# andi611/ZeroSpeech-TTS-without-T

Measured on AMD Instinct MI355X. Metric: mel-frames/sec (train_ae, seg_len=128, enc_size=1024), higher is better.
Workload: dtype bf16

## Files before the change

### include/zs_amd.h

```cpp
#ifndef ZS_AMD_H
#define ZS_AMD_H
#include <stddef.h>
#include <stdint.h>

#ifdef __cplusplus
extern "C" {
#endif

#define ZS_ABI_VERSION 1

enum { ZS_F32 = 0, ZS_BF16 = 1 };
enum { ZS_OK = 0, ZS_EINVAL = -1, ZS_ELAUNCH = -2, ZS_EWORKSPACE = -3 };
enum { ZS_PAD_ZERO = 0, ZS_PAD_REFLECT = 1 };
enum { ZS_ACT_NONE = 0, ZS_ACT_LRELU = 1, ZS_ACT_SIGMOID = 2, ZS_ACT_TANH = 3 };
enum { ZS_STORE_ROWS = 0, ZS_STORE_SPLIT2 = 1 };
enum { ZS_RES_NONE = 0, ZS_RES_IDENTITY = 1, ZS_RES_AVGPOOL2 = 2, ZS_RES_UPSAMPLE2 = 3 };

int zs_abi_version(void);
const char* zs_last_error(void);
int zs_set_option(const char* key, int value);

typedef struct {
  int32_t dtype;
  const void* A; int64_t lda; int64_t a_batch_stride;
  int32_t B, T_in, T_out;
  int32_t taps, stride, pad_left, pad_mode, gather;
  int32_t cin_pad;
  const void* W; int64_t ldw;
  int32_t N, n_pad;
  const float* bias;
  const float* pre_vec; int64_t pre_vec_ld; const int64_t* vec_idx;
  int32_t act; float slope;
  const void* dact_src; int64_t dact_ld;
  const void* add_src; int64_t add_ld; int32_t add_f32;
  void* out; int64_t ldc; int32_t out_f32; int32_t out_cols; int32_t store_mode;
  void* out2; int64_t ldc2; int32_t out2_cols; int32_t store_mode2;
  const float* vec2; int64_t vec2_ld;
  int32_t groups; int64_t a_gstride, w_gstride, out_gstride, bias_gstride;
  float* colsum; int64_t colsum_ld; int32_t colsum_col0;
  int32_t colsum_post;
  const int32_t* lengths; int32_t pad_right;
  int32_t w_in, w_out, taps_h;
} ZsGemmConv;
int zs_gemm_conv(const ZsGemmConv* p, void* stream);

typedef struct {
  int32_t dtype;
  const void* dY; int64_t ldy; int32_t y_cols;
  const void* X; int64_t ldx; int64_t x_batch_stride; int32_t x_cols;
  int32_t B, T_in, T_out;
  int32_t taps, stride, pad_left, pad_mode;
  int32_t Cout, Cin;
  float* dW; int64_t so, si, sj;
  float* db;
  int32_t co_split2; int32_t accumulate;
  int32_t splits;
  void* workspace; size_t workspace_bytes;
  int32_t w_in, w_out, taps_h;
} ZsGemmWgrad;
size_t zs_gemm_wgrad_workspace_bytes(const ZsGemmWgrad* p);
int zs_gemm_wgrad(const ZsGemmWgrad* p, void* stream);

typedef struct {
  int32_t dtype;
  const float* W; int64_t so, si, sj;
  int32_t Cout, Cin, taps;
  int32_t transpose, co_split2;
  int32_t inner_pad;
  void* dst; int64_t ldw;
  int32_t n_rows, n_cols, row_offset, col_offset;
  const int32_t* row_perm;
} ZsPackWeight;
int zs_pack_weight(const ZsPackWeight* p, void* stream);
int zs_pack_weight_batch(const ZsPackWeight* jobs, int32_t n, int32_t max_blocks, void* stream);

typedef struct {
  const float* src; float* dst;
  int32_t len, src_stride, dst_stride;
} ZsVecCopy;
int zs_copy_vec_batch(const ZsVecCopy* jobs, int32_t n, void* stream);

// ... 320 lines not shown
```

### zerospeech-tts-without-t_amd/csrc/zs_gemm.hip

```cpp
#include <stdlib.h>

#include <atomic>
#include <mutex>

#include "zs_common.h"

namespace {

constexpr int BM = 128, BN = 128, NT = 256;
constexpr int ROWB = 128;
constexpr int PITCH = 144;
constexpr int TILE_BYTES = BM * PITCH;

__device__ const uint4 zs_zero_line[8] = {};

__device__ __forceinline__ int xcd_remap(int bid, int nwg) {
  const int q = nwg >> 3, r = nwg & 7, xcd = bid & 7;
  return (xcd < r ? xcd * (q + 1) : r * (q + 1) + (xcd - r) * q) + (bid >> 3);
}

__device__ __forceinline__ int conv_src_row(int gather, int pad_mode, int stride, int pad_left, int T_in, int t,
                                            int j, bool& ok) {
  if (gather == 0) {
    int s = t * stride + j - pad_left;
// ... 513 lines not shown
  gemm_epilogue<T, NT, MI>(p, acc, reinterpret_cast<float*>(smem), M, m0, n0, wm, wn, tid, g);
}

constexpr int RBM = 256, RNT = 512;
constexpr int RSTAGE = (RBM + BN) * 128;
constexpr int RING_LDS = 3 * RSTAGE;
typedef __attribute__((ext_vector_type(4))) unsigned u32x4_t;

template <typename T, int PP>
__global__ __launch_bounds__(RNT, 2) void gemm_conv_ring_kernel(const ZsGemmConv p) {
  const Geom2 g2 = make_geom2(p.w_in, p.w_out, p.taps_h, p.T_in);
  constexpr int EPS = 16 / (int)sizeof(T);
  constexpr int KC = ROWB / (int)sizeof(T);
  extern __shared__ __attribute__((aligned(16))) unsigned char smem[];
  const int tid = threadIdx.x, lane = tid & 63, wave = __builtin_amdgcn_readfirstlane(tid >> 6);
  const int wm = wave >> 1, wn = wave & 1;
  const int g = blockIdx.z;
  const T* __restrict__ A = (const T*)p.A + (int64_t)g * p.a_gstride;
  const T* __restrict__ W = (const T*)p.W + (int64_t)g * p.w_gstride;
  const int M = p.B * p.T_out;
  const int ntn = (p.N + BN - 1) / BN;
  const int ntm = (M + RBM - 1) / RBM;
  const int wg = xcd_remap(blockIdx.x, ntm * ntn);
  constexpr int GM = 4;
  const int per_group = GM * ntn;
  const int grp = wg / per_group;
  const int gm = min(GM, ntm - grp * GM);
  const int in_g = wg - grp * per_group;
  const int m0 = (grp * GM + in_g % gm) * RBM, n0 = (in_g / gm) * BN;

  const int lrow = lane >> 3, slot = lane & 7;
  int rb[4], rt[4], lseg[4];
#pragma unroll
  for (int i = 0; i < 4; ++i) {
    const int r = wave * 32 + i * 8 + lrow;
    lseg[i] = slot ^ ((r >> 1) & 7);
    const int m = m0 + r;
    conv_row_setup(p, m, M, rb[i], rt[i]);
  }
  const int chunks_per_tap = p.cin_pad / KC;
  const T* zline = reinterpret_cast<const T*>(zs_zero_line);
  const T *pa0, *pa1, *pa2, *pa3;
  int inc0, inc1, inc2, inc3;
#define ZS_SET_TAP(i, ptr, inc)                                                                         \
  {                                                                                                     \
    bool ok = false; int srow = 0;                                                                      \
    if (rb[i] >= 0) srow = conv_src_row_g(p.gather, p.pad_mode, p.stride, p.pad_left, conv_row_tin(p, rb[i]), rt[i], tap, ok, g2); \
    ptr = ok ? (A + (int64_t)conv_row_b(p, rb[i]) * p.a_batch_stride + (int64_t)srow * p.lda + lseg[i] * EPS) : (zline + lseg[i] * EPS); \
    inc = ok ? KC : 0;                                                                                  \
  }
  const int wr0 = wave * 16 + lrow, wr1 = wave * 16 + 8 + lrow;
  const T* pw0 = W + (int64_t)(n0 + wr0) * p.ldw + (slot ^ ((wr0 >> 1) & 7)) * EPS;
  const T* pw1 = W + (int64_t)(n0 + wr1) * p.ldw + (slot ^ ((wr1 >> 1) & 7)) * EPS;
  const int nk = p.taps * chunks_per_tap;
  int tap = 0, cit = 0;
  { ZS_SET_TAP(0, pa0, inc0) ZS_SET_TAP(1, pa1, inc1) ZS_SET_TAP(2, pa2, inc2) ZS_SET_TAP(3, pa3, inc3) }
  typedef __attribute__((address_space(1))) const void* gptr_t;
  typedef __attribute__((address_space(3))) void* lptr_t;
  auto dma_piece = [&](int stage, int i) {
    unsigned char* da = smem + stage * RSTAGE + wave * 4096;
    unsigned char* db = smem + stage * RSTAGE + RBM * 128 + wave * 2048;
    if (i == 0) __builtin_amdgcn_global_load_lds((gptr_t)pa0, (lptr_t)(da), 16, 0, 0);
    else if (i == 1) __builtin_amdgcn_global_load_lds((gptr_t)pa1, (lptr_t)(da + 1024), 16, 0, 0);
    else if (i == 2) __builtin_amdgcn_global_load_lds((gptr_t)pa2, (lptr_t)(da + 2048), 16, 0, 0);
    else if (i == 3) __builtin_amdgcn_global_load_lds((gptr_t)pa3, (lptr_t)(da + 3072), 16, 0, 0);
    else if (i == 4) __builtin_amdgcn_global_load_lds((gptr_t)pw0, (lptr_t)(db), 16, 0, 0);
    else __builtin_amdgcn_global_load_lds((gptr_t)pw1, (lptr_t)(db + 1024), 16, 0, 0);
  };
  auto dma_advance = [&]() {
    pw0 += KC; pw1 += KC;
    if (++cit == chunks_per_tap) {
      cit = 0; ++tap;
      if (tap < p.taps) { ZS_SET_TAP(0, pa0, inc0) ZS_SET_TAP(1, pa1, inc1) ZS_SET_TAP(2, pa2, inc2) ZS_SET_TAP(3, pa3, inc3) }
    } else {
      pa0 += inc0; pa1 += inc1; pa2 += inc2; pa3 += inc3;
    }
  };
  auto dma = [&](int stage) {
#pragma unroll
    for (int i = 0; i < 6; ++i) dma_piece(stage, i);
    dma_advance();
  };
#undef ZS_SET_TAP

  f32x16 acc[2][2];
#pragma unroll
  for (int i = 0; i < 2; ++i)
#pragma unroll
    for (int j = 0; j < 2; ++j)
#pragma unroll
      for (int r = 0; r < 16; ++r) acc[i][j][r] = 0.f;

  const int frow = lane & 31, fh = lane >> 5, fx = (frow >> 1) & 7;
  const unsigned lds0 = (unsigned)(uintptr_t)(__attribute__((address_space(3))) unsigned char*)smem;
  const unsigned a_lane = lds0 + (unsigned)((wm * 64 + frow) * 128);
  const unsigned b_lane = lds0 + (unsigned)(RBM * 128 + (wn * 64 + frow) * 128);
// ... 592 lines not shown
          asm volatile("ds_read_b64_tr_b16 %0, %1" : "=v"(rb[st][t][hb]) : "v"(xa + off));
        }
    asm volatile("s_waitcnt lgkmcnt(0)" ::: "memory");
    __builtin_amdgcn_sched_barrier(0);
#pragma unroll
    for (int st = 0; st < 2; ++st) {
      uint4 fa[2], fb[2];
#pragma unroll
      for (int t = 0; t < 2; ++t) {
        fa[t] = make_uint4(ra[st][t][0].x, ra[st][t][0].y, ra[st][t][1].x, ra[st][t][1].y);
        fb[t] = make_uint4(rb[st][t][0].x, rb[st][t][0].y, rb[st][t][1].x, rb[st][t][1].y);
      }
#pragma unroll
      for (int mi = 0; mi < 2; ++mi)
#pragma unroll
        for (int ni = 0; ni < 2; ++ni)
          acc[mi][ni] = __builtin_amdgcn_mfma_f32_32x32x16_bf16(__builtin_bit_cast(bf16x8, fa[mi]), __builtin_bit_cast(bf16x8, fb[ni]),
                                                                acc[mi][ni], 0, 0, 0);
    }
  }
};

template <typename T>
__global__ __launch_bounds__(NT, 2) void gemm_wgrad_kernel(const ZsGemmWgrad p, int ci_tiles, int rows_per_split,
                                                          int cout_r, int cin_r) {
  const Geom2 g2 = make_geom2(p.w_in, p.w_out, p.taps_h, p.T_in);
  constexpr int EPS = 16 / (int)sizeof(T);
  constexpr int SPR = 128 / EPS;
  constexpr int LPT = (WK * SPR) / NT;
  constexpr int PITCHW = WFrag<T>::PITCHW;
  constexpr int TILEW = WK * PITCHW;
  extern __shared__ __attribute__((aligned(16))) unsigned char smem[];
  unsigned char* sY = smem;
  unsigned char* sX = smem + 2 * TILEW;

  const int tid = threadIdx.x, lane = tid & 63, wave = tid >> 6;
  const int wm = wave >> 1, wn = wave & 1;
  const int per_co = p.taps * ci_tiles;
  const int tiles = ((cout_r / 128) * per_co);
  const int vid = xcd_remap(blockIdx.x, gridDim.x);
  const int split = vid / tiles, tile = vid - split * tiles;
  const int cot = tile / per_co;
  const int rem = tile - cot * per_co;
  const int tap = rem / ci_tiles, cit = rem - tap * ci_tiles;
  const int co0 = cot * 128, ci0 = cit * 128;
  const int M = p.B * p.T_out;
  const int nsplit = gridDim.x / tiles;
  const int mbeg = split * rows_per_split;
  const int mend = min(M, mbeg + rows_per_split);
  const T* __restrict__ dY = (const T*)p.dY;
  const T* __restrict__ X = (const T*)p.X;

  int lrow[LPT], lseg[LPT], lb[LPT], lt[LPT];
#pragma unroll
  for (int i = 0; i < LPT; ++i) {
    const int idx = tid + NT * i;
    lrow[i] = idx / SPR; lseg[i] = idx - lrow[i] * SPR;
    const int m = mbeg + lrow[i];
    lb[i] = m / p.T_out; lt[i] = m - lb[i] * p.T_out;
  }
  uint4 vy[LPT], vx[LPT];
  const bool do_bias = (p.db != nullptr) && tap == 0 && cit == 0;
  float bsum[LPT][EPS];
#pragma unroll
  for (int i = 0; i < LPT; ++i)
#pragma unroll
    for (int e = 0; e < EPS; ++e) bsum[i][e] = 0.f;
  auto gload = [&](int mb) {
#pragma unroll
    for (int i = 0; i < LPT; ++i) {
// ... 72 lines not shown
  float* sC = reinterpret_cast<float*>(smem);
  __syncthreads();
#pragma unroll
  for (int mi = 0; mi < 2; ++mi)
#pragma unroll
    for (int ni = 0; ni < 2; ++ni)
#pragma unroll
      for (int r = 0; r < 16; ++r) {
        const int row = wm * 64 + mi * 32 + (r & 3) + 8 * (r >> 2) + 4 * (lane >> 5);
        const int col = wn * 64 + ni * 32 + (lane & 31);
        sC[row * CPITCH + col] = acc[mi][ni][r];
      }
  __syncthreads();
  const int cg = tid & 15, rr0 = tid >> 4;
#pragma unroll 1
  for (int it = 0; it < 8; ++it) {
    const int row = rr0 + 16 * it;
    const float4 x0 = *reinterpret_cast<const float4*>(sC + row * CPITCH + cg * 8);
    const float4 x1 = *reinterpret_cast<const float4*>(sC + row * CPITCH + cg * 8 + 4);
    float* d = slab + ((int64_t)(co0 + row) * p.taps + tap) * cin_r + ci0 + cg * 8;
    *reinterpret_cast<float4*>(d) = x0;
    *reinterpret_cast<float4*>(d + 4) = x1;
  }
}

#define ZS_DSRT(dst, addr, off) asm volatile("ds_read_b64_tr_b16 %0, %1 offset:" #off : "=v"(dst) : "v"(addr))
#define ZS_WP_READ_A(base)                                                                        \
  ZS_DSRT(ya00, sa0, base + 0);    ZS_DSRT(yb00, sa0, base + 512);  ZS_DSRT(ya01, sa1, base + 0);    ZS_DSRT(yb01, sa1, base + 512);  \
  ZS_DSRT(ya10, sa0, base + 2048); ZS_DSRT(yb10, sa0, base + 2560); ZS_DSRT(ya11, sa1, base + 2048); ZS_DSRT(yb11, sa1, base + 2560); \
  ZS_DSRT(ya20, sa0, base + 4096); ZS_DSRT(yb20, sa0, base + 4608); ZS_DSRT(ya21, sa1, base + 4096); ZS_DSRT(yb21, sa1, base + 4608); \
  ZS_DSRT(ya30, sa0, base + 6144); ZS_DSRT(yb30, sa0, base + 6656); ZS_DSRT(ya31, sa1, base + 6144); ZS_DSRT(yb31, sa1, base + 6656);
#define ZS_WP_READ_B(x, sbx)                                                                      \
  ZS_DSRT(x##a0, sbx, 0);    ZS_DSRT(x##b0, sbx, 512);  ZS_DSRT(x##a1, sbx, 2048); ZS_DSRT(x##b1, sbx, 2560); \
  ZS_DSRT(x##a2, sbx, 4096); ZS_DSRT(x##b2, sbx, 4608); ZS_DSRT(x##a3, sbx, 6144); ZS_DSRT(x##b3, sbx, 6656);
#define ZS_WP_MMA(alo, ahi, blo, bhi, c)                                                          \
  c = __builtin_amdgcn_mfma_f32_32x32x16_bf16(__builtin_bit_cast(bf16x8, make_uint4(alo.x, alo.y, ahi.x, ahi.y)), \
                                               __builtin_bit_cast(bf16x8, make_uint4(blo.x, blo.y, bhi.x, bhi.y)), c, 0, 0, 0)
#define ZS_WP_DMA(cond, src, dst)                                                                 \
  __builtin_amdgcn_sched_barrier(0);                                                              \
  if (cond) __builtin_amdgcn_global_load_lds((gptr_t)(src), (lptr_t)(dst), 16, 0, 0);             \
  __builtin_amdgcn_sched_barrier(0);
#define ZS_WP_QUAD(c0, c1, x, cond, src0, dst0, src1, dst1)                                        \
  __builtin_amdgcn_s_setprio(1);                                                                  \
  ZS_WP_MMA(ya00, yb00, x##a0, x##b0, c0); ZS_WP_MMA(ya01, yb01, x##a0, x##b0, c1);               \
  ZS_WP_DMA(cond, src0, dst0)                                                                     \
  ZS_WP_MMA(ya10, yb10, x##a1, x##b1, c0); ZS_WP_MMA(ya11, yb11, x##a1, x##b1, c1); ZS_WP_MMA(ya20, yb20, x##a2, x##b2, c0); \
// ... 192 lines not shown
      for (int r = 0; r < 16; ++r) {
        const int ro = (r & 3) + 8 * (r >> 2);
        sC[(rbase + ro) * CPITCH + cb] = c000[r];            sC[(rbase + 32 + ro) * CPITCH + cb] = c001[r];
        sC[(rbase + ro) * CPITCH + cb + 32] = c010[r];       sC[(rbase + 32 + ro) * CPITCH + cb + 32] = c011[r];
        sC[(rbase + 64 + ro) * CPITCH + cb] = c100[r];       sC[(rbase + 96 + ro) * CPITCH + cb] = c101[r];
        sC[(rbase + 64 + ro) * CPITCH + cb + 32] = c110[r];  sC[(rbase + 96 + ro) * CPITCH + cb + 32] = c111[r];
      }
    }
    __syncthreads();
    const int cg = tid & 15, rr0 = tid >> 4;
#pragma unroll 1
    for (int it = 0; it < 8; ++it) {
      const int row = rr0 + 32 * it;
      const float4 x0 = *reinterpret_cast<const float4*>(sC + row * CPITCH + cg * 8);
      const float4 x1 = *reinterpret_cast<const float4*>(sC + row * CPITCH + cg * 8 + 4);
      float* d = slab + ((int64_t)(co0 + row) * p.taps + tap) * cin_r + ci0 + h * 128 + cg * 8;
      *reinterpret_cast<float4*>(d) = x0;
      *reinterpret_cast<float4*>(d + 4) = x1;
    }
    __syncthreads();
  }
}

__global__ __launch_bounds__(256) void wgrad_reduce_kernel(const ZsGemmWgrad p, int splits, int cout_r, int cin_r) {
  const int cin4 = (p.Cin + 3) >> 2;
  const int64_t total = (int64_t)p.Cout * p.taps * cin4;
  const int64_t idx = (int64_t)blockIdx.x * blockDim.x + threadIdx.x;
  if (idx >= total) return;
  const int c4 = (int)(idx % cin4);
  const int64_t rowi = idx / cin4;
  const int j = (int)(rowi % p.taps);
  const int co = (int)(rowi / p.taps);
  const int half = p.Cout >> 1;
  const int cop = p.co_split2 ? ((co & 1) * half + (co >> 1)) : co;
  const int64_t sstride = (int64_t)cout_r * p.taps * cin_r;
  const float* ws = (const float*)p.workspace + ((int64_t)cop * p.taps + j) * cin_r + c4 * 4;
  float4 acc = make_float4(0.f, 0.f, 0.f, 0.f);
  int k = 0;
  for (; k + 8 <= splits; k += 8) {
    float4 v[8];
#pragma unroll
    for (int u = 0; u < 8; ++u) v[u] = *reinterpret_cast<const float4*>(ws + (int64_t)(k + u) * sstride);
#pragma unroll
    for (int u = 0; u < 8; ++u) { acc.x += v[u].x; acc.y += v[u].y; acc.z += v[u].z; acc.w += v[u].w; }
  }
  for (; k < splits; ++k) {
    const float4 v = *reinterpret_cast<const float4*>(ws + (int64_t)k * sstride);
    acc.x += v.x; acc.y += v.y; acc.z += v.z; acc.w += v.w;
  }
  const float r[4] = {acc.x, acc.y, acc.z, acc.w};
  float* d = p.dW + (int64_t)co * p.so + (int64_t)j * p.sj;
#pragma unroll
  for (int e = 0; e < 4; ++e) {
    const int ci = c4 * 4 + e;
    if (ci < p.Cin) {
      float* q = d + (int64_t)ci * p.si;
      *q = p.accumulate ? (*q + r[e]) : r[e];
    }
  }
  if (p.db != nullptr && c4 == 0 && j == 0) {
    const float* bs = (const float*)p.workspace + (int64_t)splits * sstride + cop;
    float t = 0.f;
    for (int q2 = 0; q2 < splits; ++q2) t += bs[(int64_t)q2 * cout_r];
    p.db[co] = p.accumulate ? (p.db[co] + t) : t;
  }
}

int env_int(const char* name, int dflt) { const char* e = getenv(name); return e ? atoi(e) : dflt; }
struct Knob {
  std::atomic<int> v{-1};
  const char* env; int dflt;
  Knob(const char* e, int d) : env(e), dflt(d) {}
  int get() {
    int x = v.load(std::memory_order_relaxed);
    if (x < 0) { x = env_int(env, dflt); if (x < 0) x = 0; v.store(x, std::memory_order_relaxed); }
    return x;
  }
  int set(int nv) { const int old = get(); v.store(nv < 0 ? 0 : nv, std::memory_order_relaxed); return old; }
};
Knob g_dma64("ZS_GEMM_DMA64", 1);
Knob g_dma64_max_tiles("ZS_GEMM_DMA64_MAX_TILES", 256);
Knob g_wgrad_p8("ZS_WGRAD_P8", 1);
Knob g_wgrad_wgs("ZS_WGRAD_WGS", 256);
Knob g_wgrad_wgs128("ZS_WGRAD_WGS128", 448);
Knob g_wgrad_slab_cost("ZS_WGRAD_SLAB_COST", 13);
Knob g_wgrad_waste("ZS_WGRAD_P8_WASTE", 135);

struct WgradPlan { int p8, splits, tile, co_tiles, ci_tiles, cout_r, cin_r, rows_per_split; };
// ... 84 lines not shown
    const int pad_r = (p->T_out - 1) * p->stride + p->taps - 1 - p->pad_left - (p->T_in - 1);
    ZS_REQUIRE(p->pad_left < p->T_in && pad_r < p->T_in,
               "zs_gemm_conv: Padding size should be less than the corresponding input dimension (pad %d/%d, T %d)",
               p->pad_left, pad_r, p->T_in);
  }
  if (p->store_mode == ZS_STORE_SPLIT2 || (p->out2 && p->store_mode2 == ZS_STORE_SPLIT2))
    ZS_REQUIRE(p->N % 2 == 0, "zs_gemm_conv: SPLIT2 needs even N");
  ZS_REQUIRE(!(p->pre_vec || p->vec2) || p->vec_idx, "zs_gemm_conv: vec_idx missing");
  ZS_REQUIRE(!p->colsum || (128 % p->T_out == 0 && p->colsum_col0 >= 0 && p->colsum_col0 < p->N && !p->bias && !p->pre_vec &&
                            p->act == ZS_ACT_NONE && p->groups <= 1),
             "zs_gemm_conv: colsum needs T_out (%d) to divide 128, 0 <= colsum_col0 < N and no bias / pre_vec / activation / groups", p->T_out);
  ZS_REQUIRE(!p->lengths || (p->gather == 0 && p->B < 65536 && p->T_in < 32768 && p->pad_right >= 0 && p->colsum == nullptr),
             "zs_gemm_conv: lengths (ragged batch) needs gather 0, B < 65536, T_in < 32768, pad_right >= 0 and no colsum");
  const int groups = p->groups > 0 ? p->groups : 1;
  const int64_t M = (int64_t)p->B * p->T_out;
  const int64_t tiles = ((M + BM - 1) / BM) * ((p->N + BN - 1) / BN);
  ZS_REQUIRE(tiles < (1ll << 31), "zs_gemm_conv: grid too large");
  dim3 grid((unsigned)tiles, 1, (unsigned)groups);
  hipStream_t s = (hipStream_t)stream;
  std::call_once(g_lds_attr_once, set_lds_attrs);
  const int use_dma = g_use_dma.get(), use_ring = g_use_ring.get(), use_p8 = g_use_p8.get(), use_pp = g_use_pp.get();
  const int64_t ring_tiles = ((M + RBM - 1) / RBM) * ((p->N + BN - 1) / BN);
  const int64_t p8_tiles = ((M + PBM - 1) / PBM) * ((p->N + PBN - 1) / PBN);
  if (use_dma && use_p8 && p->n_pad % PBN == 0 && p8_tiles >= g_p8_min_tiles.get() && p8_tiles < (1ll << 31)) {
    dim3 pgrid((unsigned)p8_tiles, 1, (unsigned)groups);
    if (p->dtype == ZS_F32) hipLaunchKernelGGL(gemm_conv_p8m16_kernel<float>, pgrid, dim3(PNT), P8_LDS, s, *p);
    else hipLaunchKernelGGL(gemm_conv_p8m16_kernel<bf16_t>, pgrid, dim3(PNT), P8_LDS, s, *p);
  } else if (use_dma && use_ring && ring_tiles >= g_ring_min_tiles.get() && ring_tiles < (1ll << 31)) {
    dim3 rgrid((unsigned)ring_tiles, 1, (unsigned)groups);
    if (use_pp) {
      if (p->dtype == ZS_F32) hipLaunchKernelGGL((gemm_conv_ring_kernel<float, 1>), rgrid, dim3(RNT), RING_LDS, s, *p);
      else hipLaunchKernelGGL((gemm_conv_ring_kernel<bf16_t, 1>), rgrid, dim3(RNT), RING_LDS, s, *p);
    } else {
      if (p->dtype == ZS_F32) hipLaunchKernelGGL((gemm_conv_ring_kernel<float, 0>), rgrid, dim3(RNT), RING_LDS, s, *p);
      else hipLaunchKernelGGL((gemm_conv_ring_kernel<bf16_t, 0>), rgrid, dim3(RNT), RING_LDS, s, *p);
    }
  } else if (use_dma) {
    const int64_t tiles64 = ((M + 63) / 64) * ((p->N + BN - 1) / BN);
    if (g_dma64.get() && tiles * 2 <= g_dma64_max_tiles.get() && tiles64 < (1ll << 31) && (p->colsum == nullptr || 64 % p->T_out == 0)) {
      dim3 g64((unsigned)tiles64, 1, (unsigned)groups);
      const size_t lds = (2 * 64 * 128 + 2 * DTILE > EPI_LDS_BYTES / 2) ? 2 * 64 * 128 + 2 * DTILE : EPI_LDS_BYTES / 2;
      if (p->dtype == ZS_F32) hipLaunchKernelGGL((gemm_conv_dma_kernel<float, 64>), g64, dim3(NT), lds, s, *p);
      else hipLaunchKernelGGL((gemm_conv_dma_kernel<bf16_t, 64>), g64, dim3(NT), lds, s, *p);
      return zs_check_launch("zs_gemm_conv");
    }
    const size_t lds = (4 * DTILE > EPI_LDS_BYTES) ? 4 * DTILE : EPI_LDS_BYTES;
// ... 13 lines not shown
  else if (key && !strcmp(key, "gemm_ring")) slot = &g_use_ring;
  else if (key && !strcmp(key, "gemm_ring_min_tiles")) slot = &g_ring_min_tiles;
  else if (key && !strcmp(key, "gemm_pp")) slot = &g_use_pp;
  else if (key && !strcmp(key, "gemm_p8")) slot = &g_use_p8;
  else if (key && !strcmp(key, "gemm_p8_min_tiles")) slot = &g_p8_min_tiles;
  else if (key && !strcmp(key, "gemm_dma64")) slot = &g_dma64;
  else if (key && !strcmp(key, "gemm_dma64_max_tiles")) slot = &g_dma64_max_tiles;
  else if (key && !strcmp(key, "wgrad_p8")) slot = &g_wgrad_p8;
  else if (key && !strcmp(key, "wgrad_wgs")) slot = &g_wgrad_wgs;
  else if (key && !strcmp(key, "wgrad_wgs128")) slot = &g_wgrad_wgs128;
  else if (key && !strcmp(key, "wgrad_slab_cost")) slot = &g_wgrad_slab_cost;
  else if (key && !strcmp(key, "wgrad_p8_waste")) slot = &g_wgrad_waste;
  if (key && !strcmp(key, "gru_persist")) return zs_gru_persist_option(value);
  if (key && !strcmp(key, "gru_wide")) return zs_gru_wide_option(value);
  if (key && !strcmp(key, "gru_spin_limit")) return zs_gru_spin_limit_option(value);
  if (key && !strcmp(key, "gl_prefetch")) return zs_gl_prefetch_option(value);
  if (key && !strcmp(key, "gl_chains")) return zs_gl_chains_option(value);
  if (key && !strcmp(key, "norm_wide")) return zs_norm_wide_option(value);
  if (key && !strncmp(key, "norm_lim", 8) && key[8] >= '0' && key[8] <= '2' && !key[9]) return zs_norm_lim_option(key[8] - '0', value);
  if (!slot) { zs_set_error("zs_set_option: unknown key %s", key ? key : "(null)"); return ZS_EINVAL; }
  return slot->set(value);
}

extern "C" size_t zs_gemm_wgrad_workspace_bytes(const ZsGemmWgrad* p) {
  if (!p) return 0;
  const WgradPlan w = wgrad_plan(p);
  return (size_t)w.splits * ((size_t)w.cout_r * p->taps * w.cin_r + w.cout_r) * sizeof(float);
}

extern "C" int zs_gemm_wgrad(const ZsGemmWgrad* p, void* stream) {
  ZS_REQUIRE(p && p->dY && p->X && p->dW && p->workspace, "zs_gemm_wgrad: null operand");
  ZS_REQUIRE(aligned16(p->workspace), "zs_gemm_wgrad: workspace must be 16-byte aligned");
  ZS_REQUIRE(p->dtype == ZS_F32 || p->dtype == ZS_BF16, "zs_gemm_wgrad: bad dtype");
  const int es = p->dtype == ZS_F32 ? 4 : 2;
  ZS_REQUIRE(p->B > 0 && p->T_in > 0 && p->T_out > 0 && p->Cout > 0 && p->Cin > 0 && p->taps > 0 && p->stride > 0,
             "zs_gemm_wgrad: bad sizes");
  ZS_REQUIRE(aligned16(p->dY) && aligned16(p->X) && (p->ldy * es) % 16 == 0 && (p->ldx * es) % 16 == 0 &&
                 (p->x_batch_stride * es) % 16 == 0 && (p->y_cols * es) % 16 == 0 && (p->x_cols * es) % 16 == 0,
             "zs_gemm_wgrad: operands must be 16-byte aligned");
  ZS_REQUIRE(p->y_cols <= p->ldy && p->x_cols <= p->ldx && p->Cout <= p->y_cols && p->Cin <= p->x_cols, "zs_gemm_wgrad: column bounds");
  ZS_REQUIRE(!p->co_split2 || p->Cout % 2 == 0, "zs_gemm_wgrad: SPLIT2 needs even Cout");
  ZS_REQUIRE(p->w_in == 0 || (p->w_in > 0 && p->w_out > 0 && p->taps_h > 0 && p->taps % p->taps_h == 0 && p->T_in % p->w_in == 0 &&
                              p->T_out % p->w_out == 0 && (int64_t)p->T_out * p->w_out < (1ll << 32)),
             "zs_gemm_wgrad: 2-D geometry (w_in %d, w_out %d, taps_h %d, taps %d, T_in %d, T_out %d)", p->w_in, p->w_out, p->taps_h, p->taps,
             p->T_in, p->T_out);
  const WgradPlan w = wgrad_plan(p);
  const int splits = w.splits, co_tiles = w.co_tiles, ci_tiles = w.ci_tiles, cout_r = w.cout_r, cin_r = w.cin_r;
  const int rows_per_split = w.rows_per_split;
  const size_t need = (size_t)splits * ((size_t)cout_r * p->taps * cin_r + cout_r) * sizeof(float);
  if (p->workspace_bytes < need) {
    zs_set_error("zs_gemm_wgrad: workspace %zu < %zu bytes", p->workspace_bytes, need);
    return ZS_EWORKSPACE;
  }
  hipStream_t s = (hipStream_t)stream;
  ZS_REQUIRE((int64_t)co_tiles * p->taps * ci_tiles * splits < (1ll << 31), "zs_gemm_wgrad: grid too large");
  dim3 grid((unsigned)(co_tiles * p->taps * ci_tiles * splits), 1, 1);
  std::call_once(g_lds_attr_once, set_lds_attrs);
  if (w.p8) {
    hipLaunchKernelGGL(gemm_wgrad_p8_kernel, grid, dim3(PNT), P8_LDS, s, *p, ci_tiles, rows_per_split, cout_r, cin_r);
  } else if (p->dtype == ZS_F32) {
    const size_t lds = (4 * WK * WFrag<float>::PITCHW > EPI_LDS_BYTES) ? 4 * WK * WFrag<float>::PITCHW : EPI_LDS_BYTES;
    hipLaunchKernelGGL(gemm_wgrad_kernel<float>, grid, dim3(NT), lds, s, *p, ci_tiles, rows_per_split, cout_r, cin_r);
  } else {
    const size_t lds = (4 * WK * WFrag<bf16_t>::PITCHW > EPI_LDS_BYTES) ? 4 * WK * WFrag<bf16_t>::PITCHW : EPI_LDS_BYTES;
    hipLaunchKernelGGL(gemm_wgrad_kernel<bf16_t>, grid, dim3(NT), lds, s, *p, ci_tiles, rows_per_split, cout_r, cin_r);
  }
  int rc = zs_check_launch("zs_gemm_wgrad");
  if (rc) return rc;
// ... 5 lines not shown
```

### zerospeech-tts-without-t_amd/engine.py

```python
import os
import torch

from . import _lib as L
from .layers import Act, ConvLayer, GruLayer, colsum_ok, fork_side, join_side, rup

LRELU = L.ZS_ACT_LRELU
EPS_IN = 1e-5
_UID = [0]


def _uid():
    _UID[0] += 1
    return _UID[0]


def _half_up(t):
    return (t + 1) // 2


GUMBEL_MODES = {'one_hot': L.ZS_ENC_ONE_HOT, 'binary': L.ZS_ENC_BINARY, 'continues': L.ZS_ENC_CONTINUES}


def linear_width(enc_mode, E):
    return {'multilabel_binary': 2 * E, 'binary': E * E}.get(enc_mode, E)


class EncoderEngine(object):
    def __init__(self, ctx, P, G, c_in, c_h1, c_h2, c_h3, enc_size, ns, dp, seg_len, enc_mode='multilabel_binary'):
        self.ctx = ctx
        self.uid = _uid()
        self.c_in, self.c1, self.c2, self.H, self.E = c_in, c_h1, c_h2, c_h3, enc_size
        self.mode = enc_mode
        self.n_lin = linear_width(enc_mode, enc_size)
        self.ns, self.dp = float(ns), float(dp)
        self.pad_mode = L.ZS_PAD_REFLECT if seg_len >= 64 else L.ZS_PAD_ZERO
        if c_h1 % 8 or c_h2 % 8:
            raise ValueError('c_h1 and c_h2 must be multiples of 8 (16-byte rows)')
        mk = lambda n, **kw: ConvLayer(ctx, P[n + '.weight'], P[n + '.bias'], G[n + '.weight'], G[n + '.bias'],
                                       pad_mode=self.pad_mode, name=n, **kw)
        self.conv1s = [mk('conv1s.%d' % i) for i in range(7)]
        self.conv2 = mk('conv2')
        self.convs = [(mk('conv%d' % a), mk('conv%d' % b, stride=2)) for a, b in ((3, 4), (5, 6), (7, 8))]
        self.dense = [(mk('dense%d' % a), mk('dense%d' % b)) for a, b in ((1, 2), (3, 4))]
        self.gru = GruLayer(ctx, P, G, 'RNN.', name='enc%d' % self.uid)
        self.linear = mk('linear')
        self.layers = self.conv1s + [self.conv2] + [l for p in self.convs for l in p] + [l for p in self.dense for l in p] + \
            [self.linear]
        self.ncat = 7 * c_h1 + c_in
        self.tape = None

    def pack(self):
        with L.pack_batch(self.ctx.stream):
            for l in self.layers:
                l.pack()
            self.gru.pack()

    def forward(self, x, training, noise=None, noise_kind=2, seed=0, drop_masks=None, seed_ptr=None, lengths=None):
        c, ns = self.ctx, self.ns
        B, T, F = x.shape
        Ls = [None] * 4
        if lengths is not None:
            if training:
                raise L.ZsError('EncoderEngine: ragged batches are an inference feature')
            l0 = torch.as_tensor(lengths, dtype=torch.int32).reshape(-1)
            if l0.numel() != B or int(l0.max()) > T or int(l0.min()) < 9:
                raise L.ZsError('EncoderEngine: lengths must be %d values in [9, %d]' % (B, T))
            l1 = (l0 + 1) // 2; l2 = (l1 + 1) // 2; l3 = (l2 + 1) // 2
            self.last_lengths = l3
            ld = torch.stack([l0, l1, l2, l3]).to(c.device, non_blocking=True)
            Ls = [ld[i] for i in range(4)]
        assert F == self.c_in and x.dtype == torch.float32 and x.is_contiguous()
        st = c.stream
        c1, c2, H, E = self.c1, self.c2, self.H, self.E
        dp = self.dp if training else 0.0
        masks = drop_masks if drop_masks is not None else [None] * 6
        Ts = [T, _half_up(T), _half_up(_half_up(T)), _half_up(_half_up(_half_up(T)))]
        T4 = Ts[3]
        tag = '_%d_%d_%d' % (self.uid, B, T)
        tp = {'B': B, 'T': T, 'Ts': Ts, 'training': training, 'seed': seed, 'masks': masks, 'dp': dp, 'seed_ptr': seed_ptr}

        xin = c.act('e_xin' + tag, B, T, F)
        cat = c.act('e_cat' + tag, B, T, self.ncat)
        L.call('zs_cast_rows', 'ZsCastRows', st, dtype=c.dt, src=L.ptr(x), ld_src=F, src_f32=1, dst=xin.ptr(), ld_dst=xin.ld,
               dst_f32=0, col_off=0, rows=B * T, cols=F, fill_cols=xin.ld, act=L.ZS_ACT_NONE,
               dst2=cat.ptr(), ld_dst2=cat.ld, col_off2=7 * c1, fill_cols2=cat.ld - 7 * c1, act2=LRELU, slope2=ns)
        if c.overlap_wgrad and B * T >= 4096:
            sts = fork_side(c.device)
            for i, l in enumerate(self.conv1s):
                with torch.cuda.stream(sts[i % len(sts)]):
                    l.fwd(xin, out=cat.sub(i * c1, c1), act=LRELU, slope=ns, lengths=Ls[0])
            join_side(c.device)
        else:
            for i, l in enumerate(self.conv1s):
                l.fwd(xin, out=cat.sub(i * c1, c1), act=LRELU, slope=ns, lengths=Ls[0])
        y2 = c.act('e_y2' + tag, B, T, c2)
        self.conv2.fwd(cat, out=y2, act=LRELU, slope=ns)
        a = c.act('e_a0' + tag, B, T, c2)
        st0 = self._in(y2, a, tp, 0, res_mode=L.ZS_RES_NONE, lengths=Ls[0])
        tp.update(xin=xin, cat=cat, y2=y2, a0=a, st0=st0, blocks=[], dense=[])
        for i, (la, lb) in enumerate(self.convs):
            ya = c.act('e_ya%d' % i + tag, B, Ts[i], c2)
            la.fwd(a, out=ya, act=LRELU, slope=ns, lengths=Ls[i])
            yb = c.act('e_yb%d' % i + tag, B, Ts[i + 1], c2)
            lb.fwd(ya, out=yb, act=LRELU, slope=ns, lengths=Ls[i])
            an = c.act('e_a%d' % (i + 1) + tag, B, Ts[i + 1], c2)
            stt = self._in(yb, an, tp, 1 + i, res_mode=L.ZS_RES_AVGPOOL2, res=a, lengths=Ls[i + 1], res_lengths=Ls[i])
            tp['blocks'].append((a, ya, yb, stt))
            a = an
        cat2 = c.act('e_cat2' + tag, B, T4, c2 + 2 * H)
# ... 108 lines not shown
            a, ya, yb, stt = tp['blocks'][i]
            dzb = c.act('e_dzb%d' % i + tag, B, Ts[i + 1], c2)
            self._in_bwd(da, yb, stt, dzb, tp)
            lb.wgrad(dzb, ya)
            gp = c.act('e_gp%d' % i + tag, B, Ts[i] + 4, c2)
            lb.dgrad(dzb, Ts[i], gp)
            dza = c.act('e_dza%d' % i + tag, B, Ts[i], c2)
            self._combine(gp, Ts[i], 2, 2, dza, dact=ya)
            la.wgrad(dza, a)
            la.dgrad(dza, Ts[i], gp)
            dn = c.act('e_da%d' % i + tag, B, Ts[i], c2)
            self._combine(gp, Ts[i], 2, 2, dn, res_mode=L.ZS_RES_AVGPOOL2, res=da)
            da = dn
        y2, cat, xin = tp['y2'], tp['cat'], tp['xin']
        dz = c.act('e_dzy2' + tag, B, T, c2)
        self._in_bwd(da, y2, tp['st0'], dz, tp)
        self.conv2.wgrad(dz, cat)
        dcat = c.act('e_dcat' + tag, B, T, self.ncat)
        self.conv2.dgrad(dz, T, dcat, dact_src=cat, slope=ns, n_cols=7 * c1)
        self._bank = (dcat, xin)

    def backward_bank(self):
        dcat, xin = self._bank
        for i, l in enumerate(self.conv1s):
            l.wgrad(dcat.sub(i * self.c1, self.c1), xin)

    def _combine(self, gp, T, pl, pr, out, res_mode=L.ZS_RES_NONE, res=None, dact=None):
        c = self.ctx
        L.call('zs_grad_combine', 'ZsGradCombine', c.stream, dtype=c.dt, gp=gp.ptr(), ldg=gp.ld, pad_left=pl, pad_right=pr,
               pad_mode=self.pad_mode, B=gp.B, T=T, C=gp.ld, res_mode=res_mode, res=(res.ptr() if res is not None else None),
               ldres=(res.ld if res is not None else 0), dact_src=(dact.ptr() if dact is not None else None),
               dact_ld=(dact.ld if dact is not None else 0), slope=self.ns, out=out.ptr(), ldo=out.ld, unshuffle=0)


class DecoderEngine(object):
    def __init__(self, ctx, P, G, c_in, c_out, c_h, c_a, ns, seg_len, output_mask=False):
        self.ctx = ctx
        self.uid = _uid()
        self.E, self.F, self.ch, self.n_spk = c_in, c_out, c_h, c_a
        self.ns = float(ns)
        self.pad_mode = L.ZS_PAD_REFLECT if seg_len >= 64 else L.ZS_PAD_ZERO
        self.out_act = L.ZS_ACT_TANH if output_mask else L.ZS_ACT_SIGMOID
        if c_h % 32:
            raise ValueError('Decoder c_h must be a multiple of 32 (got %d)' % c_h)
        mk = lambda n, **kw: ConvLayer(ctx, P[n + '.weight'], P[n + '.bias'], G[n + '.weight'], G[n + '.bias'],
                                       pad_mode=self.pad_mode, name=n, **kw)
# ... 307 lines not shown
```

### zerospeech-tts-without-t_amd/layers.py

```python
import ctypes
import os

import torch

from . import _lib as L


def colsum_ok(T):
    return T > 0 and 128 % T == 0


def rup(x, m):
    return (x + m - 1) // m * m


DTYPES = {'fp32': (L.ZS_F32, torch.float32), 'bf16': (L.ZS_BF16, torch.bfloat16)}
SLACK = 512


class Act(object):
    __slots__ = ('t', 'B', 'T', 'C', 'ld', 'off', 'cols')

    def __init__(self, t, B, T, C, ld, off=0, cols=None):
        self.t, self.B, self.T, self.C, self.ld, self.off = t, B, T, C, ld, off
# ... 264 lines not shown
        c = self.ctx
        Te = Tp + (Tp & 1)
        if out.T != Te:
            raise ValueError('stride-2 dgrad: the output needs %d rows per sample (padded domain %d rounded up to even), got %d' % (Te, Tp, out.T))
        ne = (self.k + 1) // 2
        for par, taps in ((0, ne), (1, self.k // 2)):
            kw = dict(dtype=c.dt, A=dY.ptr(), lda=dY.ld, a_batch_stride=dY.T * dY.ld, B=dY.B, T_in=dY.T, T_out=Te // 2, taps=taps,
                      stride=1, pad_left=0, pad_mode=L.ZS_PAD_ZERO, gather=1, cin_pad=self.cout_pad,
                      W=L.ptr(self.wd, par * ne * self.cout_pad), ldw=self.ldw_d, N=self.Cin, n_pad=self.n_pad_d, act=L.ZS_ACT_NONE,
                      out=out.ptr(par * out.ld), ldc=2 * out.ld, out_cols=(out_cols if out_cols is not None else min(out.cols, rup(self.Cin, 32))),
                      store_mode=L.ZS_STORE_ROWS, groups=1, out_f32=int(out_f32))
            L.call('zs_gemm_conv', 'ZsGemmConv', c.stream, **kw)
        return Tp

    def wgrad(self, dY, X, accumulate=False, bias=True):
        c = self.ctx
        es = c.es
        y_cols = min(dY.cols, rup(self.Cout, 16 // es))
        x_cols = min(X.cols, rup(self.Cin, 16 // es))
        kw = dict(dtype=c.dt, dY=dY.ptr(), ldy=dY.ld, y_cols=y_cols, X=X.ptr(), ldx=X.ld, x_batch_stride=X.T * X.ld,
                  x_cols=x_cols, B=X.B, T_in=X.T, T_out=dY.T, taps=self.k, stride=self.stride, pad_left=self.pad_l,
                  pad_mode=self.pad_mode, Cout=self.Cout, Cin=self.Cin, dW=L.ptr(self.gw), so=self.so, si=self.si, sj=self.sj,
                  db=(L.ptr(self.gb) if bias else None), co_split2=int(self.split2), accumulate=int(accumulate), splits=0)
        wgrad_call(c, kw, self.sid)


class Conv2dLayer(object):

    def __init__(self, ctx, weight, bias, gweight, gbias, stride=2, pad_mode=L.ZS_PAD_REFLECT, name='', dgrad_only=False):
        self.ctx, self.name = ctx, name
        self.w, self.b, self.gw, self.gb = weight, bias, gweight, gbias
        self.Cout, self.Cin, self.k = weight.shape[0], weight.shape[1], weight.shape[2]
        if weight.dim() != 4 or weight.shape[3] != self.k or stride not in (1, 2):
            raise ValueError('Conv2dLayer: square kernels, stride 1 or 2')
        self.stride, self.pad_mode, self.pad = stride, pad_mode, self.k // 2
        self.taps = self.k * self.k
        kc = ctx.kc
        self.cin_pad, self.cout_pad = rup(self.Cin, kc), rup(self.Cout, kc)
        self.ldw, self.n_pad, self.n_pad_d = self.taps * self.cin_pad, rup(self.Cout, 128), rup(self.Cin, 128)
        dev, tdt = ctx.device, ctx.tdt
        self.wf = None if dgrad_only else torch.zeros(self.n_pad * self.ldw + SLACK, dtype=tdt, device=dev)
        self.nt = [(self.k + 1) // 2, self.k // 2] if stride == 2 else [self.k]
        self.wd = {}
        for ph in range(len(self.nt)):
            for pw in range(len(self.nt)):
                ld = self.nt[ph] * self.nt[pw] * self.cout_pad
# ... 234 lines not shown
```

Measured before the change: 2.653 million.

## Fuse encoder conv bank into single windowed GEMM and batched wgrad launch

Packs the weights of the bank of 1-D convolutions (kernel sizes 1..n, 128 output channels each) into one shared weight matrix. The forward pass then runs as a single ring GEMM launch in which each 128-column block walks only its own tap window, so the zero-padded taps are skipped. Weight gradients for all bank members go through one batched wgrad kernel and one batched reduce kernel, replacing per-layer launches and the side-stream fork. The aim is to cut launch count and fill the GPU better on small convolutions. In exchange the code gains nibble-encoded window metadata and a tile order sorted by longest window first.

```diff
diff --git a/include/zs_amd.h b/include/zs_amd.h
--- a/include/zs_amd.h
+++ b/include/zs_amd.h
@@ -41,6 +41,7 @@
   int32_t colsum_post;
   const int32_t* lengths; int32_t pad_right;
   int32_t w_in, w_out, taps_h;
+  int32_t win_blocks, win_first, win_count, win_order;
 } ZsGemmConv;
 int zs_gemm_conv(const ZsGemmConv* p, void* stream);
 
@@ -57,6 +58,8 @@
   int32_t splits;
   void* workspace; size_t workspace_bytes;
   int32_t w_in, w_out, taps_h;
+  int32_t win_blocks, win_first, win_count;
+  const int64_t* win_out;
 } ZsGemmWgrad;
 size_t zs_gemm_wgrad_workspace_bytes(const ZsGemmWgrad* p);
 int zs_gemm_wgrad(const ZsGemmWgrad* p, void* stream);
diff --git a/zerospeech-tts-without-t_amd/csrc/zs_gemm.hip b/zerospeech-tts-without-t_amd/csrc/zs_gemm.hip
--- a/zerospeech-tts-without-t_amd/csrc/zs_gemm.hip
+++ b/zerospeech-tts-without-t_amd/csrc/zs_gemm.hip
@@ -559,12 +559,19 @@
   const int ntn = (p.N + BN - 1) / BN;
   const int ntm = (M + RBM - 1) / RBM;
   const int wg = xcd_remap(blockIdx.x, ntm * ntn);
-  constexpr int GM = 4;
+  const int GM = p.win_blocks > 0 ? (ntm + 7) / 8 : 4;
   const int per_group = GM * ntn;
   const int grp = wg / per_group;
   const int gm = min(GM, ntm - grp * GM);
   const int in_g = wg - grp * per_group;
-  const int m0 = (grp * GM + in_g % gm) * RBM, n0 = (in_g / gm) * BN;
+  const int m0 = (grp * GM + in_g % gm) * RBM;
+  int n0 = (in_g / gm) * BN, tap0 = 0, tap_end = p.taps;
+  if (p.win_blocks > 0) {
+    const int blk = (int)(((unsigned)p.win_order >> (4 * (in_g / gm))) & 15u);
+    n0 = blk * BN;
+    tap0 = (int)(((unsigned)p.win_first >> (4 * blk)) & 15u);
+    tap_end = tap0 + (int)(((unsigned)p.win_count >> (4 * blk)) & 15u);
+  }
 
   const int lrow = lane >> 3, slot = lane & 7;
   int rb[4], rt[4], lseg[4];
@@ -587,10 +594,10 @@
     inc = ok ? KC : 0;                                                                                  \
   }
   const int wr0 = wave * 16 + lrow, wr1 = wave * 16 + 8 + lrow;
-  const T* pw0 = W + (int64_t)(n0 + wr0) * p.ldw + (slot ^ ((wr0 >> 1) & 7)) * EPS;
-  const T* pw1 = W + (int64_t)(n0 + wr1) * p.ldw + (slot ^ ((wr1 >> 1) & 7)) * EPS;
-  const int nk = p.taps * chunks_per_tap;
-  int tap = 0, cit = 0;
+  const T* pw0 = W + (int64_t)(n0 + wr0) * p.ldw + (int64_t)tap0 * p.cin_pad + (slot ^ ((wr0 >> 1) & 7)) * EPS;
+  const T* pw1 = W + (int64_t)(n0 + wr1) * p.ldw + (int64_t)tap0 * p.cin_pad + (slot ^ ((wr1 >> 1) & 7)) * EPS;
+  const int nk = (tap_end - tap0) * chunks_per_tap;
+  int tap = tap0, cit = 0;
   { ZS_SET_TAP(0, pa0, inc0) ZS_SET_TAP(1, pa1, inc1) ZS_SET_TAP(2, pa2, inc2) ZS_SET_TAP(3, pa3, inc3) }
   typedef __attribute__((address_space(1))) const void* gptr_t;
   typedef __attribute__((address_space(3))) void* lptr_t;
@@ -608,7 +615,7 @@
     pw0 += KC; pw1 += KC;
     if (++cit == chunks_per_tap) {
       cit = 0; ++tap;
-      if (tap < p.taps) { ZS_SET_TAP(0, pa0, inc0) ZS_SET_TAP(1, pa1, inc1) ZS_SET_TAP(2, pa2, inc2) ZS_SET_TAP(3, pa3, inc3) }
+      if (tap < tap_end) { ZS_SET_TAP(0, pa0, inc0) ZS_SET_TAP(1, pa1, inc1) ZS_SET_TAP(2, pa2, inc2) ZS_SET_TAP(3, pa3, inc3) }
     } else {
       pa0 += inc0; pa1 += inc1; pa2 += inc2; pa3 += inc3;
     }
@@ -1247,8 +1254,8 @@
 };
 
 template <typename T>
-__global__ __launch_bounds__(NT, 2) void gemm_wgrad_kernel(const ZsGemmWgrad p, int ci_tiles, int rows_per_split,
-                                                          int cout_r, int cin_r) {
+__device__ __forceinline__ void wgrad128_body(const ZsGemmWgrad& p, int ci_tiles, int rows_per_split, int cout_r, int cin_r,
+                                              int vid, int nwg) {
   const Geom2 g2 = make_geom2(p.w_in, p.w_out, p.taps_h, p.T_in);
   constexpr int EPS = 16 / (int)sizeof(T);
   constexpr int SPR = 128 / EPS;
@@ -1263,14 +1270,13 @@
   const int wm = wave >> 1, wn = wave & 1;
   const int per_co = p.taps * ci_tiles;
   const int tiles = ((cout_r / 128) * per_co);
-  const int vid = xcd_remap(blockIdx.x, gridDim.x);
   const int split = vid / tiles, tile = vid - split * tiles;
   const int cot = tile / per_co;
   const int rem = tile - cot * per_co;
   const int tap = rem / ci_tiles, cit = rem - tap * ci_tiles;
   const int co0 = cot * 128, ci0 = cit * 128;
   const int M = p.B * p.T_out;
-  const int nsplit = gridDim.x / tiles;
+  const int nsplit = nwg / tiles;
   const int mbeg = split * rows_per_split;
   const int mend = min(M, mbeg + rows_per_split);
   const T* __restrict__ dY = (const T*)p.dY;
@@ -1389,6 +1395,27 @@
     *reinterpret_cast<float4*>(d) = x0;
     *reinterpret_cast<float4*>(d + 4) = x1;
   }
+}
+
+template <typename T>
+__global__ __launch_bounds__(NT, 2) void gemm_wgrad_kernel(const ZsGemmWgrad p, int ci_tiles, int rows_per_split,
+                                                          int cout_r, int cin_r) {
+  wgrad128_body<T>(p, ci_tiles, rows_per_split, cout_r, cin_r, xcd_remap(blockIdx.x, gridDim.x), gridDim.x);
+}
+
+constexpr int BANK_MAX = 8;
+struct WgradBank {
+  ZsGemmWgrad conv[BANK_MAX];
+  int wg0[BANK_MAX + 1], rel0[BANK_MAX + 1];
+  int splits[BANK_MAX], rows_per_split[BANK_MAX], ci_tiles[BANK_MAX], cout_r[BANK_MAX], cin_r[BANK_MAX];
+  int n;
+};
+__global__ __launch_bounds__(NT, 2) void gemm_wgrad_bank_kernel(const WgradBank b) {
+  int i = 0;
+  while (i + 1 < b.n && (int)blockIdx.x >= b.wg0[i + 1]) ++i;
+  const int nwg = b.wg0[i + 1] - b.wg0[i];
+  wgrad128_body<bf16_t>(b.conv[i], b.ci_tiles[i], b.rows_per_split[i], b.cout_r[i], b.cin_r[i],
+                        xcd_remap((int)blockIdx.x - b.wg0[i], nwg), nwg);
 }
 
 #define ZS_DSRT(dst, addr, off) asm volatile("ds_read_b64_tr_b16 %0, %1 offset:" #off : "=v"(dst) : "v"(addr))
@@ -1627,10 +1654,9 @@
   }
 }
 
-__global__ __launch_bounds__(256) void wgrad_reduce_kernel(const ZsGemmWgrad p, int splits, int cout_r, int cin_r) {
+__device__ __forceinline__ void wgrad_reduce_body(const ZsGemmWgrad& p, int splits, int cout_r, int cin_r, int64_t idx) {
   const int cin4 = (p.Cin + 3) >> 2;
   const int64_t total = (int64_t)p.Cout * p.taps * cin4;
-  const int64_t idx = (int64_t)blockIdx.x * blockDim.x + threadIdx.x;
   if (idx >= total) return;
   const int c4 = (int)(idx % cin4);
   const int64_t rowi = idx / cin4;
@@ -1669,6 +1695,18 @@
     for (int q2 = 0; q2 < splits; ++q2) t += bs[(int64_t)q2 * cout_r];
     p.db[co] = p.accumulate ? (p.db[co] + t) : t;
   }
+}
+
+__global__ __launch_bounds__(256) void wgrad_reduce_kernel(const ZsGemmWgrad p, int splits, int cout_r, int cin_r) {
+  wgrad_reduce_body(p, splits, cout_r, cin_r, (int64_t)blockIdx.x * blockDim.x + threadIdx.x);
+}
+
+__global__ __launch_bounds__(256) void wgrad_bank_reduce_kernel(const WgradBank b) {
+  const int idx = blockIdx.x * blockDim.x + threadIdx.x;
+  int i = 0;
+  while (i + 1 < b.n && idx >= b.rel0[i + 1]) ++i;
+  if (idx >= b.rel0[b.n]) return;
+  wgrad_reduce_body(b.conv[i], b.splits[i], b.cout_r[i], b.cin_r[i], idx - b.rel0[i]);
 }
 
 int env_int(const char* name, int dflt) { const char* e = getenv(name); return e ? atoi(e) : dflt; }
@@ -1799,6 +1837,28 @@
   const int use_dma = g_use_dma.get(), use_ring = g_use_ring.get(), use_p8 = g_use_p8.get(), use_pp = g_use_pp.get();
   const int64_t ring_tiles = ((M + RBM - 1) / RBM) * ((p->N + BN - 1) / BN);
   const int64_t p8_tiles = ((M + PBM - 1) / PBM) * ((p->N + PBN - 1) / PBN);
+  if (p->win_blocks != 0) {
+    ZS_REQUIRE(p->win_blocks > 0 && p->win_blocks <= 8 && p->win_blocks * 128 == p->n_pad && p->taps <= 15 && p->w_in == 0 &&
+                   groups == 1 && p->colsum == nullptr && p->store_mode != ZS_STORE_SPLIT2 && ring_tiles < (1ll << 31),
+               "zs_gemm_conv: tap windows need n_pad = 128 x win_blocks (<= 8), taps <= 15, 1-D, one group, no colsum / SPLIT2");
+    unsigned seen = 0;
+    for (int n = 0; n < p->win_blocks; ++n) {
+      const int f = ((unsigned)p->win_first >> (4 * n)) & 15u, c = ((unsigned)p->win_count >> (4 * n)) & 15u;
+      const int o = ((unsigned)p->win_order >> (4 * n)) & 15u;
+      ZS_REQUIRE(c >= 1 && f + c <= p->taps && o < p->win_blocks && !(seen & (1u << o)),
+                 "zs_gemm_conv: bad tap window of block %d (first %d, count %d, order %d)", n, f, c, o);
+      seen |= 1u << o;
+    }
+    dim3 rgrid((unsigned)ring_tiles, 1, 1);
+    if (use_pp) {
+      if (p->dtype == ZS_F32) hipLaunchKernelGGL((gemm_conv_ring_kernel<float, 1>), rgrid, dim3(RNT), RING_LDS, s, *p);
+      else hipLaunchKernelGGL((gemm_conv_ring_kernel<bf16_t, 1>), rgrid, dim3(RNT), RING_LDS, s, *p);
+    } else {
+      if (p->dtype == ZS_F32) hipLaunchKernelGGL((gemm_conv_ring_kernel<float, 0>), rgrid, dim3(RNT), RING_LDS, s, *p);
+      else hipLaunchKernelGGL((gemm_conv_ring_kernel<bf16_t, 0>), rgrid, dim3(RNT), RING_LDS, s, *p);
+    }
+    return zs_check_launch("zs_gemm_conv");
+  }
   if (use_dma && use_p8 && p->n_pad % PBN == 0 && p8_tiles >= g_p8_min_tiles.get() && p8_tiles < (1ll << 31)) {
     dim3 pgrid((unsigned)p8_tiles, 1, (unsigned)groups);
     if (p->dtype == ZS_F32) hipLaunchKernelGGL(gemm_conv_p8m16_kernel<float>, pgrid, dim3(PNT), P8_LDS, s, *p);
@@ -1858,8 +1918,64 @@
   return slot->set(value);
 }
 
+static bool bank_setup(const ZsGemmWgrad* p, WgradBank& b, size_t& need) {
+  memset(&b, 0, sizeof(b));
+  need = 0;
+  if (p->win_blocks <= 0 || p->win_blocks > BANK_MAX || !p->win_out || p->dtype != ZS_BF16 || p->w_in != 0 || p->co_split2 ||
+      p->Cout != 128 * p->win_blocks)
+    return false;
+  const int es = 2;
+  b.n = p->win_blocks;
+  for (int n = 0; n < b.n; ++n) {
+    const int f = ((unsigned)p->win_first >> (4 * n)) & 15u, c = ((unsigned)p->win_count >> (4 * n)) & 15u;
+    if (c < 1 || f + c > p->taps || f > p->pad_left) return false;
+    const int64_t* wo = p->win_out + 5 * n;
+    ZsGemmWgrad& q = b.conv[n];
+    q = *p;
+    q.win_blocks = 0; q.win_first = 0; q.win_count = 0; q.win_out = nullptr;
+    q.dY = (const char*)p->dY + (size_t)128 * n * es;
+    q.y_cols = 128; q.Cout = 128; q.taps = c; q.pad_left = p->pad_left - f;
+    q.dW = p->dW + wo[0]; q.so = wo[2]; q.si = wo[3]; q.sj = wo[4];
+    q.db = p->db ? p->db + wo[1] : nullptr;
+    q.splits = 0;
+    const WgradPlan w = wgrad_plan(&q);
+    if (w.p8) return false;
+    b.splits[n] = w.splits; b.rows_per_split[n] = w.rows_per_split; b.ci_tiles[n] = w.ci_tiles;
+    b.cout_r[n] = w.cout_r; b.cin_r[n] = w.cin_r;
+    b.wg0[n + 1] = b.wg0[n] + w.co_tiles * c * w.ci_tiles * w.splits;
+    b.rel0[n + 1] = b.rel0[n] + 128 * c * ((p->Cin + 3) / 4);
+    q.workspace = p->workspace ? (char*)p->workspace + need : nullptr;
+    need += (size_t)w.splits * ((size_t)w.cout_r * c * w.cin_r + w.cout_r) * sizeof(float);
+  }
+  return true;
+}
+
+static int wgrad_bank(const ZsGemmWgrad* p, void* stream) {
+  WgradBank b;
+  size_t need = 0;
+  ZS_REQUIRE(bank_setup(p, b, need),
+             "zs_gemm_wgrad: tap windows need bf16, 1-D, no co_split2, Cout = 128 x win_blocks (<= %d), win_out, and windows "
+             "with 1 <= count, first + count <= taps, first <= pad_left", BANK_MAX);
+  if (p->workspace_bytes < need) {
+    zs_set_error("zs_gemm_wgrad: workspace %zu < %zu bytes", p->workspace_bytes, need);
+    return ZS_EWORKSPACE;
+  }
+  hipStream_t s = (hipStream_t)stream;
+  const size_t lds = (4 * WK * WFrag<bf16_t>::PITCHW > EPI_LDS_BYTES) ? 4 * WK * WFrag<bf16_t>::PITCHW : EPI_LDS_BYTES;
+  hipLaunchKernelGGL(gemm_wgrad_bank_kernel, dim3((unsigned)b.wg0[b.n]), dim3(NT), lds, s, b);
+  const int rc = zs_check_launch("zs_gemm_wgrad");
+  if (rc) return rc;
+  hipLaunchKernelGGL(wgrad_bank_reduce_kernel, dim3((unsigned)((b.rel0[b.n] + 255) / 256)), dim3(256), 0, s, b);
+  return zs_check_launch("zs_gemm_wgrad.reduce");
+}
+
 extern "C" size_t zs_gemm_wgrad_workspace_bytes(const ZsGemmWgrad* p) {
   if (!p) return 0;
+  if (p->win_blocks != 0) {
+    WgradBank b;
+    size_t need = 0;
+    return bank_setup(p, b, need) ? need : 0;
+  }
   const WgradPlan w = wgrad_plan(p);
   return (size_t)w.splits * ((size_t)w.cout_r * p->taps * w.cin_r + w.cout_r) * sizeof(float);
 }
@@ -1880,6 +1996,7 @@
                               p->T_out % p->w_out == 0 && (int64_t)p->T_out * p->w_out < (1ll << 32)),
              "zs_gemm_wgrad: 2-D geometry (w_in %d, w_out %d, taps_h %d, taps %d, T_in %d, T_out %d)", p->w_in, p->w_out, p->taps_h, p->taps,
              p->T_in, p->T_out);
+  if (p->win_blocks != 0) return wgrad_bank(p, stream);
   const WgradPlan w = wgrad_plan(p);
   const int splits = w.splits, co_tiles = w.co_tiles, ci_tiles = w.ci_tiles, cout_r = w.cout_r, cin_r = w.cin_r;
   const int rows_per_split = w.rows_per_split;
diff --git a/zerospeech-tts-without-t_amd/engine.py b/zerospeech-tts-without-t_amd/engine.py
--- a/zerospeech-tts-without-t_amd/engine.py
+++ b/zerospeech-tts-without-t_amd/engine.py
@@ -2,7 +2,7 @@
 import torch
 
 from . import _lib as L
-from .layers import Act, ConvLayer, GruLayer, colsum_ok, fork_side, join_side, rup
+from .layers import Act, ConvBank, ConvLayer, GruLayer, colsum_ok, fork_side, join_side, rup
 
 LRELU = L.ZS_ACT_LRELU
 EPS_IN = 1e-5
@@ -47,12 +47,16 @@
         self.layers = self.conv1s + [self.conv2] + [l for p in self.convs for l in p] + [l for p in self.dense for l in p] + \
             [self.linear]
         self.ncat = 7 * c_h1 + c_in
+        self.bank = ConvBank(ctx, self.conv1s, self.pad_mode) if ConvBank.usable(ctx, self.conv1s) else None
         self.tape = None
 
     def pack(self):
         with L.pack_batch(self.ctx.stream):
             for l in self.layers:
-                l.pack()
+                if self.bank is None or l not in self.conv1s:
+                    l.pack()
+            if self.bank is not None:
+                self.bank.pack()
             self.gru.pack()
 
     def forward(self, x, training, noise=None, noise_kind=2, seed=0, drop_masks=None, seed_ptr=None, lengths=None):
@@ -84,7 +88,9 @@
         L.call('zs_cast_rows', 'ZsCastRows', st, dtype=c.dt, src=L.ptr(x), ld_src=F, src_f32=1, dst=xin.ptr(), ld_dst=xin.ld,
                dst_f32=0, col_off=0, rows=B * T, cols=F, fill_cols=xin.ld, act=L.ZS_ACT_NONE,
                dst2=cat.ptr(), ld_dst2=cat.ld, col_off2=7 * c1, fill_cols2=cat.ld - 7 * c1, act2=LRELU, slope2=ns)
-        if c.overlap_wgrad and B * T >= 4096:
+        if self.bank is not None:
+            self.bank.fwd(xin, cat.sub(0, 7 * c1), act=LRELU, slope=ns, lengths=Ls[0])
+        elif c.overlap_wgrad and B * T >= 4096:
             sts = fork_side(c.device)
             for i, l in enumerate(self.conv1s):
                 with torch.cuda.stream(sts[i % len(sts)]):
@@ -239,6 +245,9 @@
 
     def backward_bank(self):
         dcat, xin = self._bank
+        if self.bank is not None:
+            self.bank.wgrad(dcat, xin)
+            return
         for i, l in enumerate(self.conv1s):
             l.wgrad(dcat.sub(i * self.c1, self.c1), xin)
 
diff --git a/zerospeech-tts-without-t_amd/layers.py b/zerospeech-tts-without-t_amd/layers.py
--- a/zerospeech-tts-without-t_amd/layers.py
+++ b/zerospeech-tts-without-t_amd/layers.py
@@ -310,6 +310,65 @@
                   x_cols=x_cols, B=X.B, T_in=X.T, T_out=dY.T, taps=self.k, stride=self.stride, pad_left=self.pad_l,
                   pad_mode=self.pad_mode, Cout=self.Cout, Cin=self.Cin, dW=L.ptr(self.gw), so=self.so, si=self.si, sj=self.sj,
                   db=(L.ptr(self.gb) if bias else None), co_split2=int(self.split2), accumulate=int(accumulate), splits=0)
+        wgrad_call(c, kw, self.sid)
+
+
+class ConvBank(object):
+
+    @staticmethod
+    def usable(ctx, convs):
+        n = len(convs)
+        return (ctx.dtype_name == 'bf16' and 1 <= n <= 8 and all(l.Cout == 128 and l.k == i + 1 and l.stride == 1 and l.pad_l == l.k // 2
+                                                                  and l.b is not None for i, l in enumerate(convs))
+                and len({l.Cin for l in convs}) == 1)
+
+    def __init__(self, ctx, convs, pad_mode):
+        self.ctx, self.convs, self.pad_mode = ctx, convs, pad_mode
+        n = len(convs)
+        self.taps, self.pad_l, self.pad_r = n, n // 2, n - 1 - n // 2
+        self.Cin, self.N = convs[0].Cin, 128 * n
+        self.first = [self.pad_l - l.k // 2 for l in convs]
+        self.cin_pad = rup(self.Cin, ctx.kc)
+        self.ldw = self.taps * self.cin_pad
+        nib = lambda v: sum(x << (4 * i) for i, x in enumerate(v))
+        self.win_first = nib(self.first)
+        self.win_count = nib([l.k for l in convs])
+        self.win_order = nib(sorted(range(n), key=lambda i: -convs[i].k))
+        dev = ctx.device
+        self.wf = torch.zeros(self.N * self.ldw + SLACK, dtype=ctx.tdt, device=dev)
+        self.bias = torch.zeros(self.N, dtype=torch.float32, device=dev)
+        l0 = convs[0]
+        out = [[(L.ptr(l.gw) - L.ptr(l0.gw)) // 4, (L.ptr(l.gb) - L.ptr(l0.gb)) // 4, l.so, l.si, l.sj] for l in convs]
+        self.win_out = torch.tensor(out, dtype=torch.int64)
+        self.sid = next_sid()
+
+    def pack(self):
+        c = self.ctx
+        for i, l in enumerate(self.convs):
+            L.call('zs_pack_weight', 'ZsPackWeight', c.stream, dtype=c.dt, W=L.ptr(l.w), so=l.so, si=l.si, sj=l.sj, Cout=l.Cout,
+                   Cin=l.Cin, taps=l.k, co_split2=0, transpose=0, inner_pad=self.cin_pad, dst=L.ptr(self.wf), ldw=self.ldw,
+                   n_rows=128, n_cols=l.k * self.cin_pad, row_offset=128 * i, col_offset=self.first[i] * self.cin_pad)
+            L.vec_copy(self.bias[128 * i:128 * (i + 1)], l.b, c.stream)
+
+    def fwd(self, A, out, act=L.ZS_ACT_NONE, slope=0.0, lengths=None):
+        c = self.ctx
+        kw = dict(dtype=c.dt, A=A.ptr(), lda=A.ld, a_batch_stride=A.T * A.ld, B=A.B, T_in=A.T, T_out=A.T, taps=self.taps, stride=1,
+                  pad_left=self.pad_l, pad_mode=self.pad_mode, gather=0, cin_pad=self.cin_pad, W=L.ptr(self.wf), ldw=self.ldw, N=self.N,
+                  n_pad=self.N, bias=L.ptr(self.bias), act=act, slope=slope, groups=1, out=out.ptr(), ldc=out.ld, out_f32=0,
+                  store_mode=L.ZS_STORE_ROWS, out_cols=self.N, win_blocks=len(self.convs), win_first=self.win_first,
+                  win_count=self.win_count, win_order=self.win_order)
+        if lengths is not None:
+            kw.update(lengths=L.ptr(lengths), pad_right=self.pad_r)
+        L.call('zs_gemm_conv', 'ZsGemmConv', c.stream, **kw)
+
+    def wgrad(self, dY, X, accumulate=False, bias=True):
+        c = self.ctx
+        l0 = self.convs[0]
+        kw = dict(dtype=c.dt, dY=dY.ptr(), ldy=dY.ld, y_cols=self.N, X=X.ptr(), ldx=X.ld, x_batch_stride=X.T * X.ld,
+                  x_cols=min(X.cols, rup(self.Cin, 8)), B=X.B, T_in=X.T, T_out=dY.T, taps=self.taps, stride=1, pad_left=self.pad_l,
+                  pad_mode=self.pad_mode, Cout=self.N, Cin=self.Cin, dW=L.ptr(l0.gw), so=0, si=0, sj=0,
+                  db=(L.ptr(l0.gb) if bias else None), co_split2=0, accumulate=int(accumulate), splits=0,
+                  win_blocks=len(self.convs), win_first=self.win_first, win_count=self.win_count, win_out=L.ptr(self.win_out))
         wgrad_call(c, kw, self.sid)
 
 
```

New measurement: 2.701 million (median of 6 runs). +1.8%, better.
